# ChenWu98/cycle-diffusion

Hardware: AMD Instinct MI355X
Metric: images/sec, SD-v1.4 512px CycleDiffusion 100+100 steps, 1/2/4/8 MI355X (higher is better)
Workload: dtype fp16; 1 GPU; C2: Stable-Diffusion-v1.4-shaped U-Net + KL-f8 VAE, 512x512, custom_steps=99 white_box_steps=100 eta=0.1 skip 0, 1 trial, encoder scale 1, decoder CFG 3; batch_per_gpu=4, global_batch=4, parallelism=dp1, steps_per_launch_set=5, launch_set_cap=16, launch_sets_in_flight_per_gpu=1, images_in_flight_per_gpu=20, distributed=single process, weights=synthetic(seed=0)

## Files before the change

cycle-diffusion_amd/csrc/attn.hip:

```cpp
#include <stdlib.h>

#include "common.h"
#include "kernels.h"

namespace cd {

namespace {

constexpr int KT = 64;

template <int DQK, int DV, int DH, int NBUF, bool VTOK, int KG, int NWV = 4, int DBG = 0>
__global__ __launch_bounds__(64 * NWV, DV <= 96 ? (KG == 32 ? (DV <= 64 ? 4 : 3) : 2) : 1) void k_attention(AttnParams p) {
  constexpr int NT = 64 * NWV;
  constexpr int KLD = DQK + 8;
  constexpr int VLD = KT + 8;
  constexpr int NKS = DQK / 16;
  constexpr int NDT = DV / 32;
  constexpr int CPR = DQK / 8;
  constexpr int NKR = (KT * CPR + NT - 1) / NT;
  constexpr bool ONES = DH > 0;
  constexpr int VS = DV <= 32 ? 32 : (DV <= 96 ? 96 : 160);
  constexpr int CPRV = ONES ? DH / 8 + 1 : DV / 8;
  constexpr int NVR = VTOK ? (KT * CPRV + NT - 1) / NT : (DV * 8 + NT - 1) / NT;
  constexpr int VBUF = VTOK ? KT * VS : DV * VLD;
  static_assert(!ONES || (DH < DV && (DH & 7) == 0 && ((DH >> 2) & 1) == 0), "ones row placement");
  __shared__ __attribute__((aligned(16))) bf16_t Ks[NBUF][KT * KLD];
  __shared__ __attribute__((aligned(16))) bf16_t Vs[NBUF][VBUF];

  const int tid = threadIdx.x, lane = tid & 63, wave = tid >> 6;
  const int qi = lane & 31, half = lane >> 5;
  const int h = blockIdx.y, b = blockIdx.z;
  const int q0 = blockIdx.x * (32 * NWV) + wave * 32;
  const int D = ONES ? DH : p.D;

  const bf16_t* qb = p.q + (int64_t)b * p.q_bs + h * D;
  const bf16_t* kb = p.k + (int64_t)b * p.k_bs + h * D;
  const bf16_t* vtb = VTOK ? p.v + (int64_t)b * p.v_bs + h * D
                           : p.vt + ((int64_t)b * p.H + h) * (int64_t)p.vt_dpad * p.vt_tpad;

  bf16x8 qf[NKS];
  const float qsc = p.scale * 1.44269504088896340736f;
  {
    const int q = q0 + qi;
#pragma unroll
    for (int ks = 0; ks < NKS; ++ks) {
      const int d0 = ks * 16 + 8 * half;
      uint4 raw = make_uint4(0, 0, 0, 0);
      if (q < p.Tq && d0 < D) raw = *(const uint4*)(qb + (int64_t)q * p.ldq + d0);
      if (!p.q_log2) {
        float f[8];
        unpack8(raw, f);
#pragma unroll
        for (int e = 0; e < 8; ++e) f[e] *= qsc;
        raw = pack8(f);
      }
      qf[ks] = *(bf16x8*)&raw;
    }
  }

  constexpr unsigned kNoLoad = 0x80000000u;
  const unsigned k_bytes = p.Tk > 0 ? (unsigned)(((int64_t)(p.Tk - 1) * p.ldk + D) * 2) : 0u;
  const unsigned v_bytes = VTOK ? (p.Tk > 0 ? (unsigned)(((int64_t)(p.Tk - 1) * p.ldv + D) * 2) : 0u)
                                : (unsigned)((int64_t)p.vt_dpad * p.vt_tpad * 2);
  const __amdgpu_buffer_rsrc_t rs_k = __builtin_amdgcn_make_buffer_rsrc((void*)kb, 0, k_bytes, 0x00020000);
  const __amdgpu_buffer_rsrc_t rs_v = __builtin_amdgcn_make_buffer_rsrc((void*)vtb, 0, v_bytes, 0x00020000);
  unsigned k_voff[NKR], v_voff[NVR];
  int k_loff[NKR], v_loff[NVR];
  bool v_ones[NVR];
#pragma unroll
  for (int i = 0; i < NKR; ++i) {
    const int id = tid + i * NT;
    const int row = id / CPR, ch = id % CPR;
    const bool ok = id < KT * CPR && ch * 8 < D;
    k_voff[i] = ok ? (unsigned)((row * p.ldk + ch * 8) * 2) : kNoLoad;
    k_loff[i] = id < KT * CPR ? row * KLD + ch * 8 : -1;
  }
#pragma unroll
  for (int i = 0; i < NVR; ++i) {
    const int id = tid + i * NT;
    if (VTOK) {
      const int row = id / CPRV, ch = id % CPRV;
      const bool data = id < KT * CPRV && ch * 8 < D;
      v_voff[i] = data ? (unsigned)((row * p.ldv + ch * 8) * 2) : kNoLoad;
      v_loff[i] = id < KT * CPRV ? row * VS + ch * 8 : -1;
      v_ones[i] = ONES && ch * 8 == DH;
    } else {
      const int row = id >> 3, ch = id & 7;
      v_voff[i] = row < DV ? (unsigned)((row * p.vt_tpad + ch * 8) * 2) : kNoLoad;
      v_loff[i] = row < DV ? row * VLD + (ch >> 1) * 16 + (ch & 1) * 4 : -1;
      v_ones[i] = ONES && row == DH;
    }
  }
  uint4 kreg[NKR], vreg[NVR];
  auto fetch = [&](int key0) {
    const unsigned k_toff = (unsigned)(key0 * p.ldk * 2);
    const unsigned v_toff = (unsigned)(VTOK ? key0 * p.ldv * 2 : key0 * 2);
#pragma unroll
    for (int i = 0; i < NKR; ++i)
      kreg[i] = __builtin_bit_cast(uint4, __builtin_amdgcn_raw_buffer_load_b128(rs_k, k_voff[i] + k_toff, 0, 0));
#pragma unroll
    for (int i = 0; i < NVR; ++i)
      vreg[i] = __builtin_bit_cast(uint4, __builtin_amdgcn_raw_buffer_load_b128(rs_v, v_voff[i] + v_toff, 0, 0));
  };
  auto commit = [&](int buf) {
#pragma unroll
    for (int i = 0; i < NKR; ++i)
      if (k_loff[i] >= 0) *(uint4*)(&Ks[buf][k_loff[i]]) = kreg[i];
#pragma unroll
    for (int i = 0; i < NVR; ++i) {
      uint4 v = vreg[i];
      if (VTOK) {
        if (v_ones[i]) v = make_uint4(kOnePair & 0xffffu, 0, 0, 0);
        if (v_loff[i] >= 0) *(uint4*)(&Vs[buf][v_loff[i]]) = v;
      } else {
        if (v_ones[i]) v = make_uint4(kOnePair, kOnePair, kOnePair, kOnePair);
        if (v_loff[i] >= 0) {
          *(uint2*)(&Vs[buf][v_loff[i]]) = make_uint2(v.x, v.y);
          *(uint2*)(&Vs[buf][v_loff[i] + 8]) = make_uint2(v.z, v.w);
        }
      }
    }
  };
  const int vtr_off = ((4 * half + ((lane & 15) >> 2)) * VS + 16 * ((lane >> 4) & 1) + 4 * (lane & 3));

  f32x16 o[NDT];
#pragma unroll
  for (int i = 0; i < NDT; ++i)
#pragma unroll
    for (int r = 0; r < 16; ++r) o[i][r] = 0.f;
  f32x16 negm;
#pragma unroll
  for (int r = 0; r < 16; ++r) negm[r] = 0.f;
  float l_part = 0.f;
  constexpr float kDefer = 8.0f;

  const int ntiles = (p.Tk + KT - 1) / KT;
  fetch(0);
  commit(0);
  __syncthreads();
  for (int t = 0; t < ntiles; ++t) {
    const int key0 = t * KT;
    const int buf = NBUF == 2 ? (t & 1) : 0;
    const bool more = t + 1 < ntiles;
    if (more && !(DBG & 1)) fetch(key0 + KT);
    const bf16_t* Kt = Ks[(DBG & 1) ? 0 : buf];
    const bf16_t* Vt = Vs[(DBG & 1) ? 0 : buf];

#pragma unroll
    for (int g = 0; g < KT / KG; ++g) {
      constexpr int HPG = KG / 32;
      f32x16 s[HPG];
      {
        bf16x8 kf[HPG][NKS];
#pragma unroll
        for (int kh = 0; kh < HPG; ++kh)
#pragma unroll
          for (int ks = 0; ks < NKS; ++ks)
            kf[kh][ks] = *(const bf16x8*)(Kt + ((g * HPG + kh) * 32 + qi) * KLD + ks * 16 + 8 * half);
        if (KG == 64) __builtin_amdgcn_sched_barrier(0);
#pragma unroll
        for (int ks = 0; ks < NKS; ++ks)
#pragma unroll
          for (int kh = 0; kh < HPG; ++kh) {
            if constexpr (DBG & 32) {
              if (ks == 0) {
#pragma unroll
                for (int r = 0; r < 16; ++r) s[kh][r] = negm[r] + __builtin_bit_cast(float, (uint32_t)kf[kh][NKS - 1][r & 7] << 16) * 1e-30f;
              }
            } else {
              s[kh] = CD_MFMA_32x32x16(kf[kh][ks], qf[ks], ks == 0 ? negm : s[kh]);
            }
          }
      }
      if (key0 + KT > p.Tk || p.causal) {
        const int kmax = p.causal ? min(p.Tk - 1, q0 + qi) : p.Tk - 1;
#pragma unroll
        for (int kh = 0; kh < HPG; ++kh)
#pragma unroll
          for (int r = 0; r < 16; ++r) {
            const int key = key0 + (g * HPG + kh) * 32 + (r & 3) + 8 * (r >> 2) + 4 * half;
            s[kh][r] = key <= kmax ? s[kh][r] : -INFINITY;
          }
      }
      float mx = __builtin_amdgcn_fmed3f(s[HPG - 1][14], s[HPG - 1][15], INFINITY);
      if constexpr (!(DBG & 64)) {
      if (HPG == 2) {
#pragma unroll
        for (int r = 0; r < 14; r += 2)
          asm("v_max3_f32 %0, %1, %2, %3" : "=v"(mx) : "v"(mx), "v"(s[1][r]), "v"(s[1][r + 1]));
      }
#pragma unroll
      for (int r = 0; r < (HPG == 2 ? 16 : 14); r += 2)
        asm("v_max3_f32 %0, %1, %2, %3" : "=v"(mx) : "v"(mx), "v"(s[0][r]), "v"(s[0][r + 1]));
      }
      const bool first = t == 0 && g == 0;
      if (first || (!(DBG & 64) && __any(mx > kDefer))) {
        const float mxq = fmaxf(mx, __shfl_xor(mx, 32));
        float delta = first ? mxq : fmaxf(mxq, 0.f);
        delta = delta == -INFINITY ? 0.f : delta;
        const float alpha = first ? 1.f : __builtin_amdgcn_exp2f(-delta);
#pragma unroll
        for (int kh = 0; kh < HPG; ++kh)
#pragma unroll
          for (int r = 0; r < 16; ++r) s[kh][r] -= delta;
#pragma unroll
        for (int r = 0; r < 16; ++r) negm[r] -= delta;
#pragma unroll
        for (int i = 0; i < NDT; ++i)
#pragma unroll
          for (int r = 0; r < 16; ++r) o[i][r] *= alpha;
        l_part *= alpha;
      }
      uint32_t pw[HPG][8];
      float ps = 0.f;
#pragma unroll
      for (int kh = 0; kh < HPG; ++kh)
#pragma unroll
        for (int r = 0; r < 16; r += 2) {
          const float e0 = (DBG & 8) ? s[kh][r] : __builtin_amdgcn_exp2f(s[kh][r]);
          const float e1 = (DBG & 8) ? s[kh][r + 1] : __builtin_amdgcn_exp2f(s[kh][r + 1]);
          if (!ONES) ps += e0 + e1;
          pw[kh][r >> 1] = pack2_prob(e0, e1);
        }
      if (!ONES) l_part += ps;

#pragma unroll
      for (int kh = 0; kh < HPG; ++kh)
#pragma unroll
        for (int s2 = 0; s2 < 2; ++s2) {
          const uint4 praw = make_uint4(pw[kh][4 * s2], pw[kh][4 * s2 + 1], pw[kh][4 * s2 + 2], pw[kh][4 * s2 + 3]);
          const bf16x8 pf = __builtin_bit_cast(bf16x8, praw);
          const int k16 = (g * HPG + kh) * 32 + 16 * s2;
#pragma unroll
          for (int dt = 0; dt < NDT; ++dt) {
            bf16x8 vf;
            if (VTOK) {
              typedef __attribute__((address_space(3))) bf16x4* lds4_t;
              const bf16_t* vr = Vt + vtr_off + k16 * VS + dt * 32;
              const bf16x4 lo = __builtin_amdgcn_ds_read_tr16_b64_v4i16((lds4_t)vr);
              const bf16x4 hi = __builtin_amdgcn_ds_read_tr16_b64_v4i16((lds4_t)(vr + 8 * VS));
              vf = __builtin_shufflevector(lo, hi, 0, 1, 2, 3, 4, 5, 6, 7);
            } else {
              vf = *(const bf16x8*)(Vt + (dt * 32 + qi) * VLD + k16 + 8 * half);
            }
            if constexpr (DBG & 16) o[dt][0] += __builtin_bit_cast(float, (uint32_t)vf[0] << 16) * __builtin_bit_cast(float, praw.x);
            else o[dt] = CD_MFMA_32x32x16(vf, pf, o[dt]);
          }
        }
    }

    if (NBUF == 1 && !(DBG & 2)) __syncthreads();
    if (more && !(DBG & 1)) commit(NBUF == 2 ? (buf ^ 1) : 0);
    if (!(DBG & 2)) __syncthreads();
  }

  float l_tot;
  if (ONES) {
    constexpr int L = DH % 32;
    const float lv = o[DH / 32][(L & 3) + 4 * (L >> 3)];
    l_tot = __shfl(lv, qi);
  } else {
    l_tot = l_part + __shfl_xor(l_part, 32);
  }
  const float inv = 1.0f / l_tot;
  const int q = q0 + qi;
  if (q < p.Tq) {
    bf16_t* ob = p.o + (int64_t)b * p.o_bs + (int64_t)q * p.ldo + h * D;
#pragma unroll
    for (int dt = 0; dt < NDT; ++dt)
#pragma unroll
      for (int rq = 0; rq < 4; ++rq) {
        const int d0 = dt * 32 + 8 * rq + 4 * half;
        if (d0 < D) {
          float bb[4] = {0.f, 0.f, 0.f, 0.f};
          if (p.obias) {
#pragma unroll
            for (int e = 0; e < 4; ++e) bb[e] = p.obias[h * D + d0 + e];
          }
          uint2 pk;
          pk.x = pack2(o[dt][rq * 4 + 0] * inv + bb[0], o[dt][rq * 4 + 1] * inv + bb[1]);
          pk.y = pack2(o[dt][rq * 4 + 2] * inv + bb[2], o[dt][rq * 4 + 3] * inv + bb[3]);
          *(uint2*)(ob + d0) = pk;
        }
      }
  }
}

template <int NWV>
__global__ __launch_bounds__(64 * NWV, 4) void k_attention_d40(AttnParams p) {
#if defined(__HIP_DEVICE_COMPILE__)
  static_assert(NWV == 8, "one K copy per wave and tile");
  typedef __attribute__((address_space(3))) void* lptr_t;
  constexpr int D = 40, NKS = 3, ROWB = 128;
  constexpr int KBUF = KT * ROWB;
  constexpr int VBUF = 48 * ROWB;
  constexpr int BUF = KBUF + VBUF;
  __shared__ __attribute__((aligned(1024))) char lds[2 * BUF];

  const int tid = threadIdx.x, lane = tid & 63;
  const int wave = __builtin_amdgcn_readfirstlane(tid >> 6);
  const int qi = lane & 31, half = lane >> 5;
  const int h = blockIdx.y, b = blockIdx.z;
  const int q0 = blockIdx.x * (32 * NWV) + wave * 32;

  const bf16_t* qb = p.q + (int64_t)b * p.q_bs + h * D;
  const bf16_t* kb = p.k + (int64_t)b * p.k_bs + h * D;
  const bf16_t* vtb = p.vt + ((int64_t)b * p.H + h) * (int64_t)p.vt_dpad * p.vt_tpad;

  bf16x8 qf[NKS];
  {
    const float qsc = p.scale * 1.44269504088896340736f;
    const int q = q0 + qi;
#pragma unroll
    for (int ks = 0; ks < NKS; ++ks) {
      const int d0 = ks * 16 + 8 * half;
      uint4 raw = make_uint4(0, 0, 0, 0);
      if (q < p.Tq && d0 < D) raw = *(const uint4*)(qb + (int64_t)q * p.ldq + d0);
      if (!p.q_log2) {
        float f[8];
        unpack8(raw, f);
#pragma unroll
        for (int e = 0; e < 8; ++e) f[e] *= qsc;
        raw = pack8(f);
      }
      qf[ks] = *(bf16x8*)&raw;
    }
  }

  constexpr unsigned kNoLoad = 0x80000000u;
  const unsigned k_bytes = p.Tk > 0 ? (unsigned)(((int64_t)(p.Tk - 1) * p.ldk + D) * 2) : 0u;
  const unsigned v_bytes = (unsigned)((int64_t)p.vt_dpad * p.vt_tpad * 2);
  const __amdgpu_buffer_rsrc_t rs_k = __builtin_amdgcn_make_buffer_rsrc((void*)kb, 0, k_bytes, 0x00020000);
  const __amdgpu_buffer_rsrc_t rs_v = __builtin_amdgcn_make_buffer_rsrc((void*)vtb, 0, v_bytes, 0x00020000);
  unsigned k_voff, v_voff;
  {
    const int row = 8 * wave + (lane >> 3);
    const int lc = (lane & 7) ^ ((row >> 1) & 7);
    const int pc = (row >> 2) & 3;
    const int key = (row & ~12) | ((((pc & 1) << 1) | (pc >> 1)) << 2);
    k_voff = lc < D / 8 ? (unsigned)((key * p.ldk + lc * 8) * 2) : kNoLoad;
    v_voff = (row < D && row < p.vt_dpad) ? (unsigned)((row * p.vt_tpad + lc * 8) * 2) : kNoLoad;
  }
  auto fetch = [&](int key0, int buf) {
    char* kd = lds + buf * BUF + wave * 1024;
    __builtin_amdgcn_raw_ptr_buffer_load_lds(rs_k, (lptr_t)kd, 16, k_voff + (unsigned)(key0 * p.ldk * 2), 0, 0, 0);
    if (wave < D / 8)
      __builtin_amdgcn_raw_ptr_buffer_load_lds(rs_v, (lptr_t)(kd + KBUF), 16, v_voff + (unsigned)(key0 * 2), 0, 0, 0);
  };
  if (wave == 5 || wave == 6) {
    const uint4 v = lane < 8 ? make_uint4(kOnePair, kOnePair, kOnePair, kOnePair) : make_uint4(0, 0, 0, 0);
    *(uint4*)(lds + (wave - 5) * BUF + KBUF + D * ROWB + lane * 16) = v;
  }

  const int sw = (qi >> 1) & 7;
  const int kf_off = qi * ROWB;
  const int vf_off = KBUF + qi * ROWB;
  const int tm = lane & 15, tg = lane >> 4;
  const int vt_off = KBUF + (32 + tm) * ROWB;
  const int vt_sw = ((32 + tm) >> 1) & 7, vt_lc = ((tg & 1) << 1) | (tg >> 1);

  f32x16 o0;
  f32x4 ot0 = {0.f, 0.f, 0.f, 0.f}, ot1 = {0.f, 0.f, 0.f, 0.f};
  f32x16 negm;
#pragma unroll
  for (int r = 0; r < 16; ++r) { o0[r] = 0.f; negm[r] = 0.f; }
  constexpr float kDefer = 8.0f;

  const int ntiles = (p.Tk + KT - 1) / KT;
  fetch(0, 0);
  asm volatile("s_waitcnt vmcnt(0)" ::: "memory");
  __syncthreads();
  for (int t = 0; t < ntiles; ++t) {
    const int key0 = t * KT;
    const int buf = t & 1;
    if (t + 1 < ntiles) fetch(key0 + KT, buf ^ 1);
    const char* Bt = lds + buf * BUF;
#pragma unroll
    for (int g = 0; g < 2; ++g) {
      f32x16 s;
      {
        bf16x8 kf[NKS];
#pragma unroll
        for (int ks = 0; ks < NKS; ++ks)
          kf[ks] = *(const bf16x8*)(Bt + kf_off + g * 32 * ROWB + (((2 * ks + half) ^ sw) << 4));
#pragma unroll
        for (int ks = 0; ks < NKS; ++ks) s = CD_MFMA_32x32x16(kf[ks], qf[ks], ks == 0 ? negm : s);
      }
      if (key0 + KT > p.Tk || p.causal) {
        const int kmax = p.causal ? min(p.Tk - 1, q0 + qi) : p.Tk - 1;
#pragma unroll
        for (int r = 0; r < 16; ++r) {
          const int row = (r & 3) + 8 * (r >> 2) + 4 * half;
          const int pc = (row >> 2) & 3;
          const int key = key0 + g * 32 + ((row & ~12) | ((((pc & 1) << 1) | (pc >> 1)) << 2));
          s[r] = key <= kmax ? s[r] : -INFINITY;
        }
      }
      float mx = __builtin_amdgcn_fmed3f(s[14], s[15], INFINITY);
#pragma unroll
      for (int r = 0; r < 14; r += 2) asm("v_max3_f32 %0, %1, %2, %3" : "=v"(mx) : "v"(mx), "v"(s[r]), "v"(s[r + 1]));
      const bool first = t == 0 && g == 0;
      if (first || __any(mx > kDefer)) {
        const float mxq = fmaxf(mx, __shfl_xor(mx, 32));
        float delta = first ? mxq : fmaxf(mxq, 0.f);
        delta = delta == -INFINITY ? 0.f : delta;
        const float alpha = first ? 1.f : __builtin_amdgcn_exp2f(-delta);
#pragma unroll
        for (int r = 0; r < 16; ++r) { s[r] -= delta; negm[r] -= delta; o0[r] *= alpha; }
        const float a0 = __shfl(alpha, lane & 15), a1 = __shfl(alpha, 16 + (lane & 15));
#pragma unroll
        for (int r = 0; r < 4; ++r) { ot0[r] *= a0; ot1[r] *= a1; }
      }
      uint32_t pw[8];
#pragma unroll
      for (int r = 0; r < 16; r += 2)
        pw[r >> 1] = pack2_prob(__builtin_amdgcn_exp2f(s[r]), __builtin_amdgcn_exp2f(s[r + 1]));
#pragma unroll
      for (int s2 = 0; s2 < 2; ++s2) {
        const bf16x8 vf = *(const bf16x8*)(Bt + vf_off + (((4 * g + 2 * s2 + half) ^ sw) << 4));
        const uint4 praw = make_uint4(pw[4 * s2], pw[4 * s2 + 1], pw[4 * s2 + 2], pw[4 * s2 + 3]);
        o0 = CD_MFMA_32x32x16(vf, __builtin_bit_cast(bf16x8, praw), o0);
      }
      {
        uint32_t xa[4], ya[4];
#pragma unroll
        for (int i = 0; i < 4; ++i) {
          const auto r2 = __builtin_amdgcn_permlane16_swap(pw[i], pw[4 + i], false, false);
          xa[i] = r2[0]; ya[i] = r2[1];
        }
        const bf16x8 va = *(const bf16x8*)(Bt + vt_off + (((4 * g + vt_lc) ^ vt_sw) << 4));
        ot0 = CD_MFMA_16x16x32(va, __builtin_bit_cast(bf16x8, make_uint4(xa[0], xa[1], xa[2], xa[3])), ot0);
        ot1 = CD_MFMA_16x16x32(va, __builtin_bit_cast(bf16x8, make_uint4(ya[0], ya[1], ya[2], ya[3])), ot1);
      }
    }
    asm volatile("s_waitcnt vmcnt(0)" ::: "memory");
    __syncthreads();
  }

  const float l0 = __shfl(ot0[0], 32 + (lane & 15)), l1 = __shfl(ot1[0], 32 + (lane & 15));
  {
    const int q = q0 + qi;
    const float inv = 1.0f / ((qi & 16) ? l1 : l0);
    if (q < p.Tq) {
      bf16_t* ob = p.o + (int64_t)b * p.o_bs + (int64_t)q * p.ldo + h * D;
#pragma unroll
      for (int rq = 0; rq < 4; ++rq) {
        const int d0 = 8 * rq + 4 * half;
        float bb[4] = {0.f, 0.f, 0.f, 0.f};
        if (p.obias) {
#pragma unroll
          for (int e = 0; e < 4; ++e) bb[e] = p.obias[h * D + d0 + e];
        }
        uint2 pk;
        pk.x = pack2(o0[rq * 4 + 0] * inv + bb[0], o0[rq * 4 + 1] * inv + bb[1]);
        pk.y = pack2(o0[rq * 4 + 2] * inv + bb[2], o0[rq * 4 + 3] * inv + bb[3]);
        *(uint2*)(ob + d0) = pk;
      }
    }
  }
  if (tg < 2) {
    const int d0 = 32 + 4 * tg;
    float bb[4] = {0.f, 0.f, 0.f, 0.f};
    if (p.obias) {
#pragma unroll
      for (int e = 0; e < 4; ++e) bb[e] = p.obias[h * D + d0 + e];
    }
#pragma unroll
    for (int qh = 0; qh < 2; ++qh) {
      const int q = q0 + tm + 16 * qh;
      const f32x4 ov = qh ? ot1 : ot0;
      const float inv = 1.0f / (qh ? l1 : l0);
      if (q < p.Tq) {
        uint2 pk;
        pk.x = pack2(ov[0] * inv + bb[0], ov[1] * inv + bb[1]);
        pk.y = pack2(ov[2] * inv + bb[2], ov[3] * inv + bb[3]);
        *(uint2*)(p.o + (int64_t)b * p.o_bs + (int64_t)q * p.ldo + h * D + d0) = pk;
      }
    }
  }
#endif
}

__global__ __launch_bounds__(256) void k_transpose_v(const bf16_t* __restrict__ v, int ldv, int64_t v_bs,
                                                     bf16_t* __restrict__ vt, int H, int Tk, int D,
                                                     int Dpad, int Tpad) {
  extern __shared__ __attribute__((aligned(16))) bf16_t tile[];
  const int key0 = blockIdx.x * 64, h = blockIdx.y, b = blockIdx.z;
  const int ldt = D + 2;
  const int cpr = D / 8;
  for (int id = threadIdx.x; id < 64 * cpr; id += 256) {
    const int row = id / cpr, ch = id % cpr;
    uint4 raw = make_uint4(0, 0, 0, 0);
    if (key0 + row < Tk) raw = *(const uint4*)(v + (int64_t)b * v_bs + (int64_t)(key0 + row) * ldv + h * D + ch * 8);
    bf16_t* d = tile + row * ldt + ch * 8;
    const bf16_t* rs = (const bf16_t*)&raw;
#pragma unroll
    for (int e = 0; e < 8; ++e) d[e] = rs[e];
  }
  __syncthreads();
  bf16_t* ob = vt + ((int64_t)b * H + h) * (int64_t)Dpad * Tpad;
  for (int id = threadIdx.x; id < Dpad * 64; id += 256) {
    const int d = id >> 6, key = id & 63;
    bf16_t val = 0;
    if (d < D) val = tile[key * ldt + d];
    ob[(int64_t)d * Tpad + key0 + key] = val;
  }
}

}

void launch_attention(hipStream_t st, const AttnParams& p) {
  CD_CHECK(p.D % 8 == 0 && p.D <= 160, "attention: head dim %d unsupported by the fused kernel", p.D);
  CD_CHECK((p.v != nullptr) != (p.vt != nullptr), "attention: exactly one of v (token-major) / vt (transposed)");
  if (p.vt) CD_CHECK(p.vt_tpad % KT == 0 && p.vt_tpad >= round_up(p.Tk, KT), "attention: V^T key padding");
  else CD_CHECK((p.ldv % 8) == 0 && ((uintptr_t)p.v & 15) == 0, "attention: V row stride / alignment");
  CD_CHECK((p.ldq % 8) == 0 && (p.ldk % 8) == 0 && (p.ldo % 4) == 0, "attention: leading dims");
  dim3 grid(ceil_div(p.Tq, 128), p.H, p.B);
#define CD_ATTN_KG(DQK, DV, DH, NBUF, KG)                                                                    \
  do {                                                                                                      \
    if (p.v) hipLaunchKernelGGL((k_attention<DQK, DV, DH, NBUF, true, KG>), grid, dim3(256), 0, st, p);      \
    else hipLaunchKernelGGL((k_attention<DQK, DV, DH, NBUF, false, KG>), grid, dim3(256), 0, st, p);         \
  } while (0)
#define CD_ATTN(DQK, DV, DH, NBUF) CD_ATTN_KG(DQK, DV, DH, NBUF, 64)
  static const bool half_groups = [] { const char* e = getenv("CD_ATTN_KG32"); return !(e && e[0] == '0'); }();
  static const bool wide_wg = [] { const char* e = getenv("CD_ATTN_W8"); return !(e && e[0] == '0'); }();
  if (p.D == 40 && half_groups && wide_wg && p.Tq >= 1024 && p.Tk >= 1024 && p.vt) {
#ifdef CD_PROBE
    static const int dbg = [] { const char* e = getenv("CD_ATTN_DBG"); return e ? atoi(e) : 0; }();
    const dim3 g8(ceil_div(p.Tq, 256), p.H, p.B);
    static const bool timed = getenv("CD_ATTN_TIME") != nullptr;
    struct Timer {
      hipStream_t st; bool on; hipEvent_t e0, e1;
      Timer(hipStream_t s, bool o) : st(s), on(o) { if (on) { hipEventCreate(&e0); hipEventCreate(&e1); hipEventRecord(e0, st); } }
      ~Timer() {
        if (!on) return;
        hipEventRecord(e1, st); hipEventSynchronize(e1);
        float ms = 0; hipEventElapsedTime(&ms, e0, e1);
        printf("[attn d40 w8 dbg %d] %.1f us\n", dbg, ms * 1e3f);
        hipEventDestroy(e0); hipEventDestroy(e1);
      }
    } timer(st, timed);
#define CD_ATTN_DBG_CASE(V) case V: hipLaunchKernelGGL((k_attention<48, 64, 40, 2, false, 32, 8, V>), g8, dim3(512), 0, st, p); return;
    switch (dbg) {
      CD_ATTN_DBG_CASE(1) CD_ATTN_DBG_CASE(2) CD_ATTN_DBG_CASE(3) CD_ATTN_DBG_CASE(8) CD_ATTN_DBG_CASE(16) CD_ATTN_DBG_CASE(32)
      CD_ATTN_DBG_CASE(48) CD_ATTN_DBG_CASE(64) CD_ATTN_DBG_CASE(72) CD_ATTN_DBG_CASE(75) CD_ATTN_DBG_CASE(51)
      default: break;
    }
#undef CD_ATTN_DBG_CASE
#endif
    static const bool d40_new = [] { const char* e = getenv("CD_ATTN_D40"); return !(e && e[0] == '0'); }();
    const bool aligned16 = ((((uintptr_t)p.q | (uintptr_t)p.k | (uintptr_t)p.vt | (uintptr_t)p.o) & 15) == 0) &&
                           (p.ldq % 8) == 0 && (p.ldk % 8) == 0 && (p.ldo % 8) == 0 && (p.q_bs % 8) == 0 && (p.k_bs % 8) == 0 &&
                           (p.o_bs % 8) == 0;
    if (d40_new && p.vt_dpad >= 40 && aligned16 && (p.vt_tpad % 8) == 0 && p.vt_tpad >= ceil_div(p.Tk, 64) * 64 &&
        (int64_t)p.Tk * p.ldk * 2 < (1ll << 31) && (int64_t)p.vt_dpad * p.vt_tpad * 2 < (1ll << 31))
      hipLaunchKernelGGL((k_attention_d40<8>), dim3(ceil_div(p.Tq, 256), p.H, p.B), dim3(512), 0, st, p);
    else
      hipLaunchKernelGGL((k_attention<48, 64, 40, 2, false, 32, 8>), dim3(ceil_div(p.Tq, 256), p.H, p.B), dim3(512), 0, st,
                         p);
  } else if (p.D == 40 && half_groups) CD_ATTN_KG(48, 64, 40, 2, 32);
  else if (p.D == 40) CD_ATTN(48, 64, 40, 2);
  else if (p.D == 80 && half_groups) CD_ATTN_KG(80, 96, 80, 2, 32);
  else if (p.D == 80) CD_ATTN(80, 96, 80, 2);
  else if (p.D <= 32) CD_ATTN(32, 32, 0, 2);
  else if (p.D <= 48) CD_ATTN(48, 64, 0, 2);
  else if (p.D <= 64) CD_ATTN(64, 64, 0, 2);
  else if (p.D <= 80) CD_ATTN(80, 96, 0, 2);
  else if (p.D <= 96) CD_ATTN(96, 96, 0, 2);
  else if (p.D <= 128) CD_ATTN(128, 128, 0, 1);
  else CD_ATTN(160, 160, 0, 1);
#undef CD_ATTN
#undef CD_ATTN_KG
}

void launch_transpose_v(hipStream_t st, const bf16_t* v, int ldv, int64_t v_bs, bf16_t* vt, int B,
                        int H, int Tk, int D, int Dpad, int Tpad) {
  CD_CHECK(D % 8 == 0 && Tpad % 64 == 0, "transpose_v: D %% 8, Tpad %% 64");
  const size_t lds = (size_t)64 * (D + 2) * sizeof(bf16_t);
  hipLaunchKernelGGL(k_transpose_v, dim3(Tpad / 64, H, B), dim3(256), lds, st, v, ldv, v_bs, vt, H,
                     Tk, D, Dpad, Tpad);
}

}
```

Before: 3.403 images/s.

## Rewrite d40 attention main loop with precomputed LDS offsets and integer max

Adds a new default main-loop variant for the head-dim-40 attention kernel. It precomputes swizzled LDS addresses, hoists the mask bounds out of the loop and unrolls the loop two tiles at a time so the buffer index is a compile-time constant. It also inserts a scheduling barrier and computes the running row max as an integer max over float bits, which is meant to shorten the softmax critical path. The integer max is only valid for non-negative scores, so the first tile falls back to a float max. The old loop stays reachable via an environment variable.

```diff
diff --git a/cycle-diffusion_amd/csrc/attn.hip b/cycle-diffusion_amd/csrc/attn.hip
--- a/cycle-diffusion_amd/csrc/attn.hip
+++ b/cycle-diffusion_amd/csrc/attn.hip
@@ -8,6 +8,21 @@
 namespace {
 
 constexpr int KT = 64;
+
+__device__ __forceinline__ int score_bits(float x) { return __builtin_bit_cast(int, x); }
+__device__ __forceinline__ int imax3(int a, int b, int c) { return max(max(a, b), c); }
+__device__ __forceinline__ int group_max_bits(const f32x16& s) {
+  int m = imax3(score_bits(s[0]), score_bits(s[1]), score_bits(s[2]));
+#pragma unroll
+  for (int r = 3; r < 15; r += 2) m = imax3(m, score_bits(s[r]), score_bits(s[r + 1]));
+  return max(m, score_bits(s[15]));
+}
+__device__ __forceinline__ float group_max_float(const f32x16& s) {
+  float m = s[0];
+#pragma unroll
+  for (int r = 1; r < 16; ++r) m = fmaxf(m, s[r]);
+  return m;
+}
 
 template <int DQK, int DV, int DH, int NBUF, bool VTOK, int KG, int NWV = 4, int DBG = 0>
 __global__ __launch_bounds__(64 * NWV, DV <= 96 ? (KG == 32 ? (DV <= 64 ? 4 : 3) : 2) : 1) void k_attention(AttnParams p) {
@@ -182,19 +197,18 @@
             s[kh][r] = key <= kmax ? s[kh][r] : -INFINITY;
           }
       }
-      float mx = __builtin_amdgcn_fmed3f(s[HPG - 1][14], s[HPG - 1][15], INFINITY);
+      float mx = 0.f;
       if constexpr (!(DBG & 64)) {
-      if (HPG == 2) {
-#pragma unroll
-        for (int r = 0; r < 14; r += 2)
-          asm("v_max3_f32 %0, %1, %2, %3" : "=v"(mx) : "v"(mx), "v"(s[1][r]), "v"(s[1][r + 1]));
-      }
-#pragma unroll
-      for (int r = 0; r < (HPG == 2 ? 16 : 14); r += 2)
-        asm("v_max3_f32 %0, %1, %2, %3" : "=v"(mx) : "v"(mx), "v"(s[0][r]), "v"(s[0][r + 1]));
+        int mb = group_max_bits(s[0]);
+        if (HPG == 2) mb = max(mb, group_max_bits(s[1]));
+        mx = __builtin_bit_cast(float, mb);
       }
       const bool first = t == 0 && g == 0;
       if (first || (!(DBG & 64) && __any(mx > kDefer))) {
+        if (first) {
+          mx = group_max_float(s[0]);
+          if (HPG == 2) mx = fmaxf(mx, group_max_float(s[1]));
+        }
         const float mxq = fmaxf(mx, __shfl_xor(mx, 32));
         float delta = first ? mxq : fmaxf(mxq, 0.f);
         delta = delta == -INFINITY ? 0.f : delta;
@@ -286,8 +300,8 @@
   }
 }
 
-template <int NWV>
-__global__ __launch_bounds__(64 * NWV, 4) void k_attention_d40(AttnParams p) {
+template <int NWV, int LOOP>
+__device__ __forceinline__ void attention_d40_body(const AttnParams& p) {
 #if defined(__HIP_DEVICE_COMPILE__)
   static_assert(NWV == 8, "one K copy per wave and tile");
   typedef __attribute__((address_space(3))) void* lptr_t;
@@ -370,6 +384,86 @@
   fetch(0, 0);
   asm volatile("s_waitcnt vmcnt(0)" ::: "memory");
   __syncthreads();
+  if constexpr (LOOP == 6) {
+    int kf_a[NKS], vf_a[4], vt_a[2];
+#pragma unroll
+    for (int ks = 0; ks < NKS; ++ks) kf_a[ks] = kf_off + (((2 * ks + half) ^ sw) << 4);
+#pragma unroll
+    for (int c = 0; c < 4; ++c) vf_a[c] = vf_off + (((2 * c + half) ^ sw) << 4);
+#pragma unroll
+    for (int g = 0; g < 2; ++g) vt_a[g] = vt_off + (((4 * g + vt_lc) ^ vt_sw) << 4);
+    const int mask_from = p.causal ? 0 : p.Tk - KT + 1;
+    const int kmax = p.causal ? min(p.Tk - 1, q0 + qi) : p.Tk - 1;
+    auto tile = [&](const int t, const int buf, const bool t0) __attribute__((always_inline)) {
+      const int key0 = t * KT;
+      if (t + 1 < ntiles) fetch(key0 + KT, buf ^ 1);
+      const char* Bt = lds + buf * BUF;
+#pragma unroll
+      for (int g = 0; g < 2; ++g) {
+        f32x16 s;
+        {
+          bf16x8 kf[NKS];
+#pragma unroll
+          for (int ks = 0; ks < NKS; ++ks) kf[ks] = *(const bf16x8*)(Bt + g * 32 * ROWB + kf_a[ks]);
+#pragma unroll
+          for (int ks = 0; ks < NKS; ++ks) s = CD_MFMA_32x32x16(kf[ks], qf[ks], ks == 0 ? negm : s);
+        }
+        if (key0 >= mask_from) {
+#pragma unroll
+          for (int r = 0; r < 16; ++r) {
+            const int row = (r & 3) + 8 * (r >> 2) + 4 * half;
+            const int pc = (row >> 2) & 3;
+            const int key = key0 + g * 32 + ((row & ~12) | ((((pc & 1) << 1) | (pc >> 1)) << 2));
+            s[r] = key <= kmax ? s[r] : -INFINITY;
+          }
+        }
+        float mx = __builtin_bit_cast(float, group_max_bits(s));
+        const bool first = t0 && g == 0 && t == 0;
+        if (first || __any(mx > kDefer)) {
+          if (first) mx = group_max_float(s);
+          const float mxq = fmaxf(mx, __shfl_xor(mx, 32));
+          float delta = first ? mxq : fmaxf(mxq, 0.f);
+          delta = delta == -INFINITY ? 0.f : delta;
+          const float alpha = first ? 1.f : __builtin_amdgcn_exp2f(-delta);
+#pragma unroll
+          for (int r = 0; r < 16; ++r) { s[r] -= delta; negm[r] -= delta; o0[r] *= alpha; }
+          const float a0 = __shfl(alpha, lane & 15), a1 = __shfl(alpha, 16 + (lane & 15));
+#pragma unroll
+          for (int r = 0; r < 4; ++r) { ot0[r] *= a0; ot1[r] *= a1; }
+        }
+        uint32_t pw[8];
+#pragma unroll
+        for (int r = 0; r < 16; r += 2)
+          pw[r >> 1] = pack2_prob(__builtin_amdgcn_exp2f(s[r]), __builtin_amdgcn_exp2f(s[r + 1]));
+#pragma unroll
+        for (int s2 = 0; s2 < 2; ++s2) {
+          const bf16x8 vf = *(const bf16x8*)(Bt + vf_a[2 * g + s2]);
+          const uint4 praw = make_uint4(pw[4 * s2], pw[4 * s2 + 1], pw[4 * s2 + 2], pw[4 * s2 + 3]);
+          o0 = CD_MFMA_32x32x16(vf, __builtin_bit_cast(bf16x8, praw), o0);
+        }
+        __builtin_amdgcn_sched_barrier(0);
+        {
+          uint32_t xa[4], ya[4];
+#pragma unroll
+          for (int i = 0; i < 4; ++i) {
+            const auto r2 = __builtin_amdgcn_permlane16_swap(pw[i], pw[4 + i], false, false);
+            xa[i] = r2[0]; ya[i] = r2[1];
+          }
+          const bf16x8 va = *(const bf16x8*)(Bt + vt_a[g]);
+          ot0 = CD_MFMA_16x16x32(va, __builtin_bit_cast(bf16x8, make_uint4(xa[0], xa[1], xa[2], xa[3])), ot0);
+          ot1 = CD_MFMA_16x16x32(va, __builtin_bit_cast(bf16x8, make_uint4(ya[0], ya[1], ya[2], ya[3])), ot1);
+        }
+      }
+      asm volatile("s_waitcnt vmcnt(0)" ::: "memory");
+      __syncthreads();
+    };
+    int t = 0;
+    for (; t + 1 < ntiles; t += 2) {
+      tile(t, 0, true);
+      tile(t + 1, 1, false);
+    }
+    if (t < ntiles) tile(t, 0, true);
+  } else {
   for (int t = 0; t < ntiles; ++t) {
     const int key0 = t * KT;
     const int buf = t & 1;
@@ -435,6 +529,7 @@
     }
     asm volatile("s_waitcnt vmcnt(0)" ::: "memory");
     __syncthreads();
+  }
   }
 
   const float l0 = __shfl(ot0[0], 32 + (lane & 15)), l1 = __shfl(ot1[0], 32 + (lane & 15));
@@ -479,6 +574,16 @@
     }
   }
 #endif
+}
+
+template <int NWV>
+__global__ __launch_bounds__(64 * NWV, 4) void k_attention_d40(AttnParams p) {
+  attention_d40_body<NWV, 6>(p);
+}
+
+template <int NWV>
+__global__ __launch_bounds__(64 * NWV, 4) void k_attention_d40_r5(AttnParams p) {
+  attention_d40_body<NWV, 5>(p);
 }
 
 __global__ __launch_bounds__(256) void k_transpose_v(const bf16_t* __restrict__ v, int ldv, int64_t v_bs,
@@ -548,14 +653,18 @@
     }
 #undef CD_ATTN_DBG_CASE
 #endif
-    static const bool d40_new = [] { const char* e = getenv("CD_ATTN_D40"); return !(e && e[0] == '0'); }();
+    static const int d40_sel = [] { const char* e = getenv("CD_ATTN_D40"); return e ? atoi(e) : 6; }();
+    const bool d40_new = d40_sel != 0;
     const bool aligned16 = ((((uintptr_t)p.q | (uintptr_t)p.k | (uintptr_t)p.vt | (uintptr_t)p.o) & 15) == 0) &&
                            (p.ldq % 8) == 0 && (p.ldk % 8) == 0 && (p.ldo % 8) == 0 && (p.q_bs % 8) == 0 && (p.k_bs % 8) == 0 &&
                            (p.o_bs % 8) == 0;
     if (d40_new && p.vt_dpad >= 40 && aligned16 && (p.vt_tpad % 8) == 0 && p.vt_tpad >= ceil_div(p.Tk, 64) * 64 &&
         (int64_t)p.Tk * p.ldk * 2 < (1ll << 31) && (int64_t)p.vt_dpad * p.vt_tpad * 2 < (1ll << 31))
-      hipLaunchKernelGGL((k_attention_d40<8>), dim3(ceil_div(p.Tq, 256), p.H, p.B), dim3(512), 0, st, p);
-    else
+    {
+      const dim3 g8(ceil_div(p.Tq, 256), p.H, p.B);
+      if (d40_sel == 5) hipLaunchKernelGGL((k_attention_d40_r5<8>), g8, dim3(512), 0, st, p);
+      else hipLaunchKernelGGL((k_attention_d40<8>), g8, dim3(512), 0, st, p);
+    } else
       hipLaunchKernelGGL((k_attention<48, 64, 40, 2, false, 32, 8>), dim3(ceil_div(p.Tq, 256), p.H, p.B), dim3(512), 0, st,
                          p);
   } else if (p.D == 40 && half_groups) CD_ATTN_KG(48, 64, 40, 2, 32);
```

Result: no change. 3.428 images/s (median of 6 runs) (+0.8%).
